# epfl-lts2/pygsp

Measured on AMD Instinct MI355X. Metric: filtered-vertices/sec (N·Nsig·K/s) + achieved HBM GB/s vs roofline, 1M-vertex K=30, higher is better.
Workload: dtype f64

## Files before the change

### pygsp_amd/csrc/gspx_ctx.hip.h

```cpp
#pragma once

struct Options {
  int64_t kernel = 0;
  int64_t vec = 0;
  int64_t rows_per_wave = 0;
  int64_t narrow_g_log2 = -1;
  int64_t waves_per_block = 4;
  int64_t calib_mix = 0;
  int64_t graph_launch = 2;
  int64_t tile_gather = 1;
  int64_t tile_workgroups = 0;
  int64_t knn_f32 = 1;
  int64_t tile_pad = 1;
  int64_t tile_min_row = 16;
  int64_t staged_copy = 1;
  int64_t staged_copy_min_mb = 32;
  int64_t copy_threads = 0;
  int64_t tile_regroup = 1;
  int64_t tile_lg = 0;
  int64_t edge_vertex_walk = 1;
  int64_t fuse_input = 1;
  int64_t tile_nt = -1;
  int64_t synthesis = 0;
  int64_t alternate_sweep = 1;
  int64_t xcd_remap = 1;
  int64_t combine = 0;
  int64_t ws_limit_mb = 65536;
  int64_t max_batch = 0;
  int64_t gather_rccl = 1;
  int64_t lds_pad_kb = 0;
  int64_t host_pipeline = 1;
  int64_t host_batch = 0;
  int64_t host_edge = 0;
  int64_t host_threads = 0;
  int64_t streamed_alloc = 1;
};

struct gspx_ctx {
  int device = 0;
  int cu_count = 256;
  hipStream_t stream = nullptr;
  Options opt;
  DevMem ws_t;
  DevMem ws_r;
  DevMem ws_w;
  DevMem io_x, io_y;
  DevMem ws_spec;
  DevMem ws_sq, ws_sqp;
  HostPipe* pipe = nullptr;
  CopyStage* copy = nullptr;
  bool counted = false;
  std::mutex comms_mu;
  std::vector<struct gspx_comm*> comms;
  hipEvent_t ev[4] = {nullptr, nullptr, nullptr, nullptr};
// ... 27 lines not shown
}

struct gspx_buf {
  gspx_ctx* ctx = nullptr;
  DevMem mem;
  int64_t bytes = 0;
};

static std::atomic<uint64_t> g_generation{1};

struct gspx_graph {
  gspx_ctx* ctx = nullptr;
  const uint64_t generation = g_generation.fetch_add(1);
  int64_t N = 0;
  int dtype = GSPX_F64;
  bool from_w = false;
  int64_t nnz_l = 0;
  DevMem lptr, lcol, lval, dw;
  int64_t nnz_int = 0;
  DevMem rptr, rcol, rval, fval, coff;
  unsigned coff_ldb = 0;
  DevMem perm, iperm;
  bool has_perm = false;
  double fval_lmax = -1.0;
  double build_ms = 0.0;
  bool has_bounds = false;
  double bounds[4] = {0, 0, 0, 0};
  DevMem gt_hdr, gt_s1rows, gt_lidx;
  DevMem gt_s1nat;
  int gt_ns1 = 0;
  int gt_rows = 0, gt_nb = 0, gt_slow = 0;
  size_t gt_lds = 0;
  int gt_entmax = 0;
  int lap_type = GSPX_LAP_COMBINATORIAL;
  bool edges_built = false;
  int64_t n_edges = 0;
  DevMem e_off, e_toff, e_src, e_dst, e_tedge, e_cs, e_ct, e_w;
};

static size_t elt_size(int dtype) { return dtype == GSPX_F32 ? 4 : 8; }

static hipEvent_t pool_event(gspx_ctx* ctx, size_t& i_ref) {
  size_t i = i_ref - 1;
  if (i >= 1024) {
    i = 1020 + (i & 3);
    i_ref = i + 1;
  }
  while (ctx->ev_pool.size() <= i) {
    hipEvent_t e = nullptr;
    if (hipEventCreate(&e) != hipSuccess) return nullptr;
    ctx->ev_pool.push_back(e);
  }
  return ctx->ev_pool[i];
}

extern "C" int gspx_device_count(int* n) {
  if (!n) return set_err(GSPX_ERR_INVALID, "gspx_device_count: null output");
  int c = 0;
  hipError_t e = hipGetDeviceCount(&c);
  if (e != hipSuccess) {
    *n = 0;
    (void)hipGetLastError();
    return set_err(GSPX_ERR_NODEVICE, "hipGetDeviceCount failed: %s", hipGetErrorString(e));
  }
  *n = c;
  return GSPX_OK;
// ... 100 lines not shown
}

struct OptionDef {
  const char* key;
  int64_t Options::*slot;
  bool (*ok)(int64_t);
  const char* refusal;
};
static const OptionDef OPTION_TABLE[] = {
    {"kernel", &Options::kernel, [](int64_t v) { return v == 0 || v == 1 || v == 2 || v == 5; },
     "kernel must be 0 (auto), 1 (panel), 2 (narrow) or 5 (LDS-staged)"},
    {"vec", &Options::vec, [](int64_t v) { return v == 0 || v == 1 || v == 2 || v == 4; }, "vec must be 0, 1, 2 or 4"},
    {"rows_per_wave", &Options::rows_per_wave, [](int64_t v) { return v >= 0 && v <= 1024; },
     "rows_per_wave must be in [0, 1024] (0 = auto)"},
    {"narrow_g_log2", &Options::narrow_g_log2, [](int64_t v) { return v >= -1 && v <= 6; },
     "narrow_g_log2 must be in [-1, 6] (-1 = auto)"},
    {"waves_per_block", &Options::waves_per_block, [](int64_t v) { return v == 4 || v == 8 || v == 16; },
     "waves_per_block must be 4, 8 or 16"},
    {"alternate_sweep", &Options::alternate_sweep, nullptr, nullptr},
    {"synthesis", &Options::synthesis, nullptr, nullptr},
    {"tile_gather", &Options::tile_gather, nullptr, nullptr},
    {"graph_launch", &Options::graph_launch, nullptr, nullptr},
    {"tile_workgroups", &Options::tile_workgroups, nullptr, nullptr},
    {"tile_lg", &Options::tile_lg, nullptr, nullptr},
    {"tile_regroup", &Options::tile_regroup, nullptr, nullptr},
    {"staged_copy", &Options::staged_copy, nullptr, nullptr},
    {"staged_copy_min_mb", &Options::staged_copy_min_mb, nullptr, nullptr},
    {"copy_threads", &Options::copy_threads, nullptr, nullptr},
    {"tile_min_row", &Options::tile_min_row, nullptr, nullptr},
    {"tile_pad", &Options::tile_pad, nullptr, nullptr},
    {"knn_f32", &Options::knn_f32, nullptr, nullptr},
    {"tile_nt", &Options::tile_nt, nullptr, nullptr},
    {"fuse_input", &Options::fuse_input, nullptr, nullptr},
    {"edge_vertex_walk", &Options::edge_vertex_walk, nullptr, nullptr},
    {"xcd_remap", &Options::xcd_remap, nullptr, nullptr},
    {"combine", &Options::combine, nullptr, nullptr},
    {"ws_limit_mb", &Options::ws_limit_mb, nullptr, nullptr},
    {"max_batch", &Options::max_batch, nullptr, nullptr},
    {"gather_rccl", &Options::gather_rccl, nullptr, nullptr},
    {"lds_pad_kb", &Options::lds_pad_kb, nullptr, nullptr},
    {"host_pipeline", &Options::host_pipeline, nullptr, nullptr},
    {"host_batch", &Options::host_batch, nullptr, nullptr},
    {"host_edge", &Options::host_edge, nullptr, nullptr},
    {"host_threads", &Options::host_threads, nullptr, nullptr},
    {"streamed_alloc", &Options::streamed_alloc, nullptr, nullptr},
};

static const OptionDef* find_option(const char* key) {
  if (key)
    for (const OptionDef& d : OPTION_TABLE)
      if (!strcmp(key, d.key)) return &d;
  set_err(GSPX_ERR_INVALID, "unknown option '%s'", key ? key : "(null)");
  return nullptr;
}

extern "C" int gspx_ctx_set_option(gspx_ctx* ctx, const char* key, int64_t value) {
  replay_reset(ctx);
  if (!ctx) return set_err(GSPX_ERR_INVALID, "null ctx");
  const OptionDef* d = find_option(key);
  if (!d) return GSPX_ERR_INVALID;
  if (d->ok && !d->ok(value)) return set_err(GSPX_ERR_INVALID, "%s", d->refusal);
  ctx->opt.*d->slot = value;
  if (d->slot == &Options::streamed_alloc) {
    const bool on = value != 0;
    (void)hipSetDevice(ctx->device);
    for (DevMem* m : {&ctx->ws_t, &ctx->ws_r}) {
// ... 186 lines not shown
```

### pygsp_amd/csrc/gspx_graph.hip.h

```cpp
#pragma once

namespace gspx {

#define GSPX_SCAN_TILE 1024
__global__ __launch_bounds__(256) void k_scan_tiles(const int* in, int n, int* out, int* __restrict__ tile_sums) {
  __shared__ int wsum[4];
  const int t = threadIdx.x, lane = t & 63, wv = t >> 6;
  const int base = blockIdx.x * GSPX_SCAN_TILE + t * 4;
  int v[4];
#pragma unroll
  for (int k = 0; k < 4; ++k) v[k] = (base + k < n) ? in[base + k] : 0;
  const int mine = v[0] + v[1] + v[2] + v[3];
  int incl = mine;
#pragma unroll
  for (int off = 1; off < 64; off <<= 1) {
    const int o = __shfl_up(incl, off);
    if (lane >= off) incl += o;
  }
  if (lane == 63) wsum[wv] = incl;
  __syncthreads();
  int wbase = 0;
  for (int k = 0; k < wv; ++k) wbase += wsum[k];
  int run = wbase + incl - mine;
#pragma unroll
// ... 615 lines not shown
  for (int i = 0; i < 4; ++i) out[i] = g->bounds[i];
  return GSPX_OK;
}

extern "C" int gspx_graph_download_internal(gspx_graph* g, int32_t* rowptr, int32_t* col) {
  if (!g || !rowptr) return set_err(GSPX_ERR_INVALID, "null argument");
  if (g->nnz_int > 0 && !col) return set_err(GSPX_ERR_INVALID, "null argument");
  HIPCHK(hipSetDevice(g->ctx->device));
  HIPCHK(hipMemcpy(rowptr, g->rptr.p, (size_t)(g->N + 1) * sizeof(int), hipMemcpyDeviceToHost));
  if (g->nnz_int > 0)
    HIPCHK(hipMemcpy(col, g->rcol.p, (size_t)g->nnz_int * sizeof(int), hipMemcpyDeviceToHost));
  return GSPX_OK;
}

extern "C" int gspx_graph_set_gather_tiles(gspx_graph* g, int block_rows, int nb, const int32_t* s1ptr,
                                           const int32_t* s1rows, const uint16_t* lidx, int64_t* stats) {
  if (g) replay_reset(g->ctx);
  if (!g) return set_err(GSPX_ERR_INVALID, "null graph");
  if (block_rows == 0) {
    g->gt_rows = 0;
    return GSPX_OK;
  }
  if (block_rows != GSPX_TILE_BR)
    return set_err(GSPX_ERR_INVALID, "gather tiles must use %d-row blocks", GSPX_TILE_BR);
  if (!s1ptr || !s1rows || !lidx || nb < 1 || nb != (int)((g->N + block_rows - 1) / block_rows))
    return set_err(GSPX_ERR_INVALID, "gspx_graph_set_gather_tiles: bad argument");
  HIPCHK(hipSetDevice(g->ctx->device));
  std::vector<int> rp((size_t)g->N + 1);
  HIPCHK(hipMemcpy(rp.data(), g->rptr.p, ((size_t)g->N + 1) * sizeof(int), hipMemcpyDeviceToHost));
  for (auto& r : rp) r &= ~3;
  const size_t lds = (size_t)52 * 1024;
  const size_t esz = elt_size(g->dtype);
  std::vector<int> hdr((size_t)nb * 4);
  int slow = 0, entmax = 0;
  for (int b = 0; b < nb; ++b) {
    const int lo = s1ptr[b], n1 = s1ptr[b + 1] - lo;
    const int r0 = b * block_rows, r1 = (int)std::min<int64_t>((int64_t)r0 + block_rows, g->N);
    const int ent = rp[r1] - rp[r0];
    if (n1 < 0 || lo < 0) return set_err(GSPX_ERR_INVALID, "gspx_graph_set_gather_tiles: bad s1ptr");
    for (int o = lo; o < lo + n1; ++o)
      if (s1rows[o] < 0 || s1rows[o] >= g->N)
        return set_err(GSPX_ERR_INVALID, "gspx_graph_set_gather_tiles: bad S1 row");
    const size_t need = (size_t)n1 * 256 + (((size_t)ent * esz + 15) & ~(size_t)15) +
                        (((size_t)ent * 2 + 15) & ~(size_t)15) + 32;
    const bool fast = n1 <= GSPX_TILE_MAXN1 && n1 < 65535 && need <= lds;
    slow += !fast;
    if (fast) entmax = std::max(entmax, ent);
    hdr[(size_t)b * 4 + 0] = lo;
    hdr[(size_t)b * 4 + 1] = fast ? n1 : -1;
    hdr[(size_t)b * 4 + 2] = rp[r0];
    hdr[(size_t)b * 4 + 3] = ent;
  }
  const int n_s1 = s1ptr[nb];
  CHK(g->gt_hdr.alloc(hdr.size() * 4 + 64));
  CHK(g->gt_s1rows.alloc((size_t)std::max(n_s1, 1) * 4 + 64));
  CHK(g->gt_lidx.alloc((size_t)g->nnz_int + 128));
  HIPCHK(hipMemcpy(g->gt_hdr.p, hdr.data(), hdr.size() * 4, hipMemcpyHostToDevice));
  HIPCHK(hipMemcpy(g->gt_s1rows.p, s1rows, (size_t)n_s1 * 4, hipMemcpyHostToDevice));
  {
    std::vector<unsigned char> l8((size_t)g->nnz_int);
    for (int b = 0; b < nb; ++b) {
      const bool fast = hdr[(size_t)b * 4 + 1] >= 0;
      const int e0 = hdr[(size_t)b * 4 + 2], e1 = e0 + hdr[(size_t)b * 4 + 3];
      for (int e = e0; e < e1; ++e) {
        if (fast && lidx[e] >= 256) return set_err(GSPX_ERR_INVALID, "gspx_graph_set_gather_tiles: tile position out of range");
        l8[(size_t)e] = fast ? (unsigned char)lidx[e] : 0;
      }
    }
    HIPCHK(hipMemcpy(g->gt_lidx.p, l8.data(), l8.size(), hipMemcpyHostToDevice));
  }
  g->gt_rows = block_rows;
  g->gt_nb = nb;
  g->gt_ns1 = n_s1;
  g->gt_s1nat.release();
  g->gt_slow = slow;
  g->gt_lds = lds;
  g->gt_entmax = entmax;
  if (stats) {
    stats[0] = nb;
    stats[1] = slow;
    stats[2] = (int64_t)lds;
  }
  return GSPX_OK;
}

static int build_tiles_dev(gspx_graph* g, size_t lds, DevMem& hdr, DevMem& s1rows, DevMem& lidx, int* out_nb, int* out_ns1,
                           int* out_slow, int* out_entmax) {
  gspx_ctx* ctx = g->ctx;
  hipStream_t st = ctx->stream;
  const int N = (int)g->N;
  constexpr int BR = GSPX_TILE_BR;
  const int nb = (N + BR - 1) / BR;
  DevMem tmp, n1, keep, s1lo, nslow;
  CHK(tmp.alloc((size_t)nb * GSPX_TILE_TMPCAP * sizeof(int)));
  CHK(n1.alloc(((size_t)nb + 1) * sizeof(int)));
  CHK(keep.alloc(((size_t)nb + 1) * sizeof(int)));
  CHK(s1lo.alloc(((size_t)nb + 1) * sizeof(int)));
  CHK(nslow.alloc(sizeof(int)));
  HIPCHK(hipMemsetAsync(nslow.p, 0, sizeof(int), st));
  hipLaunchKernelGGL(k_tiles_unique, dim3(nb), dim3(256), 0, st, g->rptr.as<int>(), g->rcol.as<int>(), N, nb,
                     tmp.as<int>(), n1.as<int>());
  hipLaunchKernelGGL(k_tiles_keep, dim3((nb + 1 + 255) / 256), dim3(256), 0, st, n1.as<int>(), nb,
                     keep.as<int>());
  CHK(scan_exclusive(ctx, keep.as<int>(), s1lo.as<int>(), nb + 1));
  int n_s1 = 0;
  HIPCHK(hipMemcpyAsync(&n_s1, s1lo.as<int>() + nb, sizeof(int), hipMemcpyDeviceToHost, st));
  HIPCHK(hipStreamSynchronize(st));
  CHK(hdr.alloc((size_t)nb * 4 * sizeof(int) + 64));
  CHK(s1rows.alloc((size_t)std::max(n_s1, 1) * 4 + 64));
  CHK(lidx.alloc((size_t)g->nnz_int + 128));
  hipLaunchKernelGGL(k_tiles_fill, dim3(nb), dim3(256), 0, st, g->rptr.as<int>(), g->rcol.as<int>(), N, nb,
                     tmp.as<int>(), n1.as<int>(), s1lo.as<int>(), (int)elt_size(g->dtype), (int)lds,
                     s1rows.as<int>(), lidx.as<unsigned char>(), hdr.as<int>(), nslow.as<int>());
  int slow = 0, entmax = 0;
  HIPCHK(hipMemcpyAsync(&slow, nslow.p, sizeof(int), hipMemcpyDeviceToHost, st));
  HIPCHK(hipMemsetAsync(nslow.p, 0, sizeof(int), st));
  hipLaunchKernelGGL(k_tiles_entmax, dim3((nb + 255) / 256), dim3(256), 0, st, hdr.as<int>(), nb, nslow.as<int>());
  HIPCHK(hipMemcpyAsync(&entmax, nslow.p, sizeof(int), hipMemcpyDeviceToHost, st));
  HIPCHK(hipGetLastError());
  HIPCHK(hipStreamSynchronize(st));
  *out_nb = nb;
  *out_ns1 = n_s1;
  *out_slow = slow;
  *out_entmax = entmax;
  return GSPX_OK;
}

extern "C" int gspx_graph_build_gather_tiles(gspx_graph* g, int64_t* stats) {
  if (!g) return set_err(GSPX_ERR_INVALID, "null graph");
  replay_reset(g->ctx);
  HIPCHK(hipSetDevice(g->ctx->device));
  if (g->N < 1) return set_err(GSPX_ERR_INVALID, "empty graph");
  const size_t lds = (size_t)52 * 1024;
  int nb = 0, n_s1 = 0, slow = 0, entmax = 0;
  CHK(build_tiles_dev(g, lds, g->gt_hdr, g->gt_s1rows, g->gt_lidx, &nb, &n_s1, &slow, &entmax));
  g->gt_rows = GSPX_TILE_BR;
  g->gt_nb = nb;
  g->gt_ns1 = n_s1;
  g->gt_s1nat.release();
  g->gt_slow = slow;
  g->gt_lds = lds;
  g->gt_entmax = entmax;
  if (stats) {
    stats[0] = nb;
    stats[1] = slow;
    stats[2] = (int64_t)lds;
    stats[3] = n_s1;
  }
  return GSPX_OK;
}

template <typename T> static int ensure_factor(gspx_graph* g, double lmax) {
  if (g->fval_lmax == lmax) return GSPX_OK;
  gspx_ctx* ctx = g->ctx;
  const int N = (int)g->N;
  const T a1 = (T)(lmax / 2.0), a2 = (T)(lmax / 2.0);
  const T two_over_a1 = T(2) / a1;
  const int nb = std::max(1, (N + 255) / 256);
  if (N > 0)
    hipLaunchKernelGGL((k_factor<T>), dim3(nb), dim3(256), 0, ctx->stream, g->rptr.as<int>(),
                       g->rcol.as<int>(), g->rval.as<T>(), N, two_over_a1, a2, g->fval.as<T>());
  HIPCHK(hipGetLastError());
  g->fval_lmax = lmax;
  return GSPX_OK;
}

__global__ void k_s1nat(const int* __restrict__ s1, const int* __restrict__ perm, int n, int* __restrict__ nat) {
  const int i = blockIdx.x * 256 + threadIdx.x;
  if (i < n) nat[i] = perm[s1[i]];
}
static int ensure_s1nat(gspx_graph* g, hipStream_t st) {
  if (g->gt_s1nat.p || !g->has_perm) return GSPX_OK;
  CHK(g->gt_s1nat.alloc((size_t)std::max(g->gt_ns1, 1) * 4 + 64));
  if (g->gt_ns1 > 0)
    hipLaunchKernelGGL(k_s1nat, dim3((g->gt_ns1 + 255) / 256), dim3(256), 0, st, g->gt_s1rows.as<int>(),
// ... 4 lines not shown
```

### pygsp_amd/csrc/gspx_poly.hip.h

```cpp
#pragma once

struct PlanStep {
  double scale = 1.0, gamma = -1.0;
  int flush = 0;
  int final = 0;
  std::vector<double> w;
};

static void make_plan_fused(int nf, int M, const std::vector<double>& cp, bool acc_existing,
                            bool final_to_y, std::vector<PlanStep>& plan) {
  const int K = M - 1;
  plan.assign((size_t)K, PlanStep());
  int covered = -1;
  bool first = !acc_existing;
  for (int k = 1; k <= K; ++k) {
    PlanStep& st = plan[(size_t)k - 1];
    st.scale = (k == 1) ? 0.5 : 1.0;
    st.gamma = (k == 1) ? 0.0 : -1.0;
    st.w.assign((size_t)nf * 3, 0.0);
    const bool must = (k == K) || (k >= 2 && (k - 2) > covered);
    if (!must) continue;
    st.flush = first ? 1 : 2;
    first = false;
    st.final = (k == K && final_to_y) ? 1 : 0;
// ... 306 lines not shown
       k_step_tile<T, 1, 4, true, false, 256>, k_step_tile<T, 1, 8, true>},
      {k_step_tile<T, 1, 1, false, true, 64>, k_step_tile<T, 1, 2, false, true, 128>,
       k_step_tile<T, 1, 4, false, true, 256>, k_step_tile<T, 1, 8, false, true>}};
  kern_t kern = narrow ? slim[flavour][lg == 1 ? 0 : lg == 2 ? 1 : lg == 4 ? 2 : 3] : wide[flavour][ncol <= 2 ? ncol : 0];
  unsigned threads = narrow ? 64u * (unsigned)lg : 512u;
  bool mix = false;
  if (opt.calib_mix && !narrow && flavour == 0) {
    static const kern_t mixk[2][3] = {
        {k_step_tile<T, 0, 16, false, false, 512, 16, 1>, k_step_tile<T, 1, 16, false, false, 512, 16, 1>,
         k_step_tile<T, 2, 16, false, false, 512, 16, 1>},
        {k_step_tile<T, 0, 16, false, false, 512, 16, 2>, k_step_tile<T, 1, 16, false, false, 512, 16, 2>,
         k_step_tile<T, 2, 16, false, false, 512, 16, 2>}};
    kern = mixk[opt.calib_mix == 2 ? 1 : 0][ncol <= 2 ? ncol : 0];
    mix = true;
  }
  const int pieces = (int)(rowb / 16);
  if (opt.tile_regroup && ncol == 1 && flavour != 1 && pieces < lg && !mix) {
#define GSPX_CL(LG_, CL_, NT_) \
  (flavour == 2 ? (kern_t)k_step_tile<T, 1, LG_, false, true, NT_, CL_> : (kern_t)k_step_tile<T, 1, LG_, false, false, NT_, CL_>)
    kern_t k2 = nullptr;
    unsigned nt2 = 0;
    if (lg == 4 && pieces == 3) k2 = GSPX_CL(4, 3, 192), nt2 = 192;
    else if (lg == 8 && pieces == 5) k2 = GSPX_CL(8, 5, 320), nt2 = 320;
    else if (lg == 16 && pieces == 10) k2 = GSPX_CL(16, 10, 320), nt2 = 320;
#undef GSPX_CL
    if (k2) kern = k2, threads = nt2;
  }
  size_t lds = g->gt_lds;
  if (lg < 8)
    lds = std::min(lds, (size_t)GSPX_TILE_MAXN1 * 16 * lg + (((size_t)g->gt_entmax * sizeof(T) + 15) & ~(size_t)15) +
                            (((size_t)g->gt_entmax + 15) & ~(size_t)15) + 64);
  if (lg < 8) lds = (lds + 2047) & ~(size_t)2047;
  int per_cu = 2;
  {
    struct Known { size_t attr = 0; std::map<size_t, int> fit; };
    static std::map<std::pair<const void*, int>, Known> known;
    static std::mutex lds_mu;
    std::lock_guard<std::mutex> lock(lds_mu);
    Known& k = known[std::make_pair((const void*)kern, g->ctx->device)];
    if (k.attr < lds) {
      HIPCHK(hipFuncSetAttribute((const void*)kern, hipFuncAttributeMaxDynamicSharedMemorySize, (int)lds));
      k.attr = lds;
    }
    if (lg < 8) {
      auto it = k.fit.find(lds);
      if (it == k.fit.end()) {
        int fit = 2;
        HIPCHK(hipOccupancyMaxActiveBlocksPerMultiprocessor(&fit, (const void*)kern, (int)threads, lds));
        it = k.fit.emplace(lds, std::max(2, std::min(fit, 16))).first;
      }
      per_cu = it->second;
    }
  }
  t.rowptr = g->rptr.as<int>();
  t.col = g->rcol.as<int>();
  t.val = vals ? vals : g->fval.as<T>();
  t.hdr = g->gt_hdr.as<int>();
  if (!t.s1rows) t.s1rows = g->gt_s1rows.as<int>();
  t.lidx = g->gt_lidx.as<unsigned char>();
  t.N = (int)g->N;
  t.ld = ld;
  t.panel_bytes = (unsigned)((size_t)g->N * ld * sizeof(T));
  t.val_bytes = (unsigned)((size_t)g->nnz_int * sizeof(T));
  t.lidx_bytes = (unsigned)((size_t)g->nnz_int);
  t.nb = g->gt_nb;
  t.ncol = ncol;
  t.per_xcd = (t.nb + 7) / 8;
  t.lds_bytes = (int)lds;
  unsigned nwg = (unsigned)std::max<int64_t>(8, ((int64_t)per_cu * g->ctx->cu_count) / 8 * 8);
  if (opt.tile_workgroups > 0)
    nwg = (unsigned)std::max<int64_t>(8, std::min<int64_t>(opt.tile_workgroups, 1 << 20) / 8 * 8);
  nwg = std::min(nwg, 8u * (unsigned)std::max(t.per_xcd, 1));
  t.nt = opt.tile_nt >= 0 ? (int)opt.tile_nt : ((size_t)g->N * ld * sizeof(T) >= ((size_t)192 << 20) ? 5 : 0);
  hipLaunchKernelGGL(kern, dim3(nwg), dim3(threads), lds, st, t);
  return GSPX_OK;
}

template <typename T>
static int prepare_coff(gspx_graph* g, const Shape& shape, unsigned ld, hipStream_t st) {
  if (shape.kernel == 5 && g->coff_ldb != ld * (unsigned)sizeof(T)) {
    CHK(g->coff.ensure(((size_t)g->nnz_int + 64) * sizeof(unsigned)));
    const int nb = std::max(1, (int)((g->N + 255) / 256));
    hipLaunchKernelGGL((k_coff<T>), dim3(nb), dim3(256), 0, st, g->rptr.as<int>(), g->rcol.as<int>(), (int)g->N,
                       ld * (unsigned)sizeof(T), g->coff.as<unsigned>());
    g->coff_ldb = ld * (unsigned)sizeof(T);
// ... 309 lines not shown
      a.gamma = T(0);
    } else {
      a.cur = B[(k + 1) & 1];
      a.out = B[k & 1];
      const bool has_b2 = (k + 2 <= K);
      a.old = has_b2 ? B[k & 1] : a.cur;
      a.gamma = has_b2 ? T(-1) : T(0);
      a.scale = (k == 0) ? T(0.5) : T(1);
    }
    a.reverse = (opt.alternate_sweep && (k & 1)) ? 1 : 0;
    launch_step<T>(a, shape, opt, st, g->coff.as<unsigned>());
  }
  HIPCHK(hipEventRecord(ev[2], st));
  if (padded) {
    const unsigned nbp = (unsigned)std::min<size_t>(((size_t)N * ld + 255) / 256, 65536);
    hipLaunchKernelGGL((k_permute_out_pad<T>), dim3(nbp), dim3(256), 0, st, B[0], ldw, y, ldy, ld, N, perm);
  }
  HIPCHK(hipEventRecord(ev[3], st));
  HIPCHK(hipGetLastError());
  return GSPX_OK;
}

template <typename T>
static int run_program_batch(gspx_graph* g, int S, const double* sc, const double* be, const double* ga, bool old_is_x,
                             const T* x, unsigned ldx, T* y, unsigned ldy, unsigned ld, size_t& ev_idx) {
  gspx_ctx* ctx = g->ctx;
  Options opt = ctx->opt;
  hipStream_t st = ctx->stream;
  const int N = (int)g->N;
  const size_t U = (size_t)N * ld;
  const Shape shape = choose_shape(opt, sizeof(T), ld, vec_cap(4, ldy, y));
  const int* perm = g->has_perm ? g->perm.as<int>() : nullptr;

  const T hw[3] = {T(1), T(0), T(0)};
  CHK(ctx->ws_w.ensure(sizeof(hw) + 64));
  HIPCHK(hipMemcpyAsync(ctx->ws_w.p, hw, sizeof(hw), hipMemcpyHostToDevice, st));
  HIPCHK(hipStreamSynchronize(st));
  CHK(ctx->ws_t.ensure((old_is_x ? 3 : 2) * U * sizeof(T) + 256));
  T* X = ctx->ws_t.as<T>();
  T* H[2] = {X + U, old_is_x ? X + 2 * U : X};

  hipEvent_t ev[4];
  CHK(batch_events(ctx, ev_idx, ev));
  launch_permute_in<T>(x, ldx, X, ld, N, perm, vec_cap(shape.vec, ldx, x), st);
  HIPCHK(hipEventRecord(ev[1], st));

  CHK(prepare_coff<T>(g, shape, ld, st));
  StepArgs<T> a = step_base<T>(g, ld, y, ldy);
  a.nf = 1;
  a.racc = H[0];
  a.wts = ctx->ws_w.as<T>();
  const bool tile_ok = tile_usable<T>(g, opt, ld, y, ldy);
  for (int s = 0; s < S; ++s) {
    const bool last = s == S - 1;
    const T* cur = (s == 0) ? X : H[(s - 1) & 1];
    T* out = H[s & 1];
    const T* old = old_is_x ? X : (const T*)out;
    const double gam = (!old_is_x && s == 0) ? 0.0 : ga[s];
    if (tile_ok) {
      TileArgs<T> t{};
      t.cur = cur;
      t.old = gam == 0.0 ? cur : old;
      t.out = out;
      t.racc = H[0];
      t.y = y;
      t.ldy = ldy;
      t.perm = perm;
      t.scale = (T)sc[s];
      t.beta = (T)be[s];
      t.gamma = (T)gam;
      t.flush = 0;
      t.final = last ? 1 : 0;
      t.reverse = (opt.alternate_sweep && (s & 1)) ? 1 : 0;
      CHK(launch_step_tile<T>(g, opt, t, ld, st));
      continue;
    }
    a.cur = cur;
    a.old = gam == 0.0 ? cur : old;
    a.out = out;
    a.scale = (T)sc[s];
    a.beta = (T)be[s];
    a.gamma = (T)gam;
    a.flush = last ? 1 : 0;
    a.final = last ? 1 : 0;
    a.reverse = (opt.alternate_sweep && (s & 1)) ? 1 : 0;
    launch_step<T>(a, shape, opt, st, g->coff.as<unsigned>());
  }
  HIPCHK(hipEventRecord(ev[2], st));
  HIPCHK(hipEventRecord(ev[3], st));
  HIPCHK(hipGetLastError());
  return GSPX_OK;
}

template <typename T>
static int filter_dev_t(gspx_graph* g, double lmax, int Nf, int M, const double* coeffs,
                        int64_t Nsig, const T* x, T* y, int mode) {
  gspx_ctx* ctx = g->ctx;
  const Options& opt = ctx->opt;
  const int64_t N = g->N;
  for (int i = 0; i < 5; ++i) ctx->timing[i] = 0;
  if (N == 0 || Nsig == 0) return GSPX_OK;
  CHK(ensure_factor<T>(g, lmax));
  std::vector<double> cp;
  halve_c0(Nf, M, coeffs, cp);

  const int K = M - 1;
// ... 347 lines not shown
```

### pygsp_amd/csrc/gspx_tile_kernels.hip.h

```cpp
#pragma once

#include "gspx_kernels.hip.h"

namespace gspx {

template <typename T> struct TileArgs {
  const int* rowptr;
  const int* col;
  const T* val;
  const int* hdr;
  const int* s1rows;
  const u8* lidx;
  const T* cur;
  const T* old;
  const int* old_rows;
  T* out;
  T* racc;
  T* y;
  const int* perm;
  int N;
  u32 ld, ldy;
  u32 panel_bytes, val_bytes, lidx_bytes;
  int nb, ncol, per_xcd;
  int lds_bytes;
  T scale, gamma;
  T beta;
  T wn, wc, wo;
  const T* inp;
  const T* wts;
  int nin;
  int flush;
  int final;
  int reverse;
  int nt;
};

constexpr int GSPX_TILE_BR = 64;
constexpr int GSPX_TILE_MAXN1 = 160;

template <typename T, int NCOL, int LG, bool OLDNAT> struct TileSchedule {
  static constexpr bool PF = !OLDNAT;
  static constexpr bool TILE_LAST = PF && LG == 16;
  static constexpr bool PF_ENTRIES = PF;
  static constexpr bool META_AFTER = !OLDNAT && LG == 16 && NCOL == 0;
};

template <typename T, int NCOL, int LG = 16, bool OLDNAT = false, bool INS = false, int NT = 512, int CL = LG,
          int MIX = 0>
__global__ __launch_bounds__(NT, 4) void k_step_tile(const TileArgs<T> a) {
  static_assert(NT == 512 || (NT == 64 * LG && NCOL == 1) || (CL < LG && NCOL == 1 && NT % 64 == 0 && NT % CL == 0),
                "narrow builds: one row per group, one chunk per row");
  constexpr int BR = GSPX_TILE_BR;
  static_assert(CL <= LG && (BR % (NT / CL)) == 0, "compute groups must tile the block's rows");
  constexpr int MAXN1 = GSPX_TILE_MAXN1;
  constexpr bool PF = TileSchedule<T, NCOL, LG, OLDNAT>::PF;
  constexpr bool META_AFTER = TileSchedule<T, NCOL, LG, OLDNAT>::META_AFTER;
  constexpr bool TILE_LAST = TileSchedule<T, NCOL, LG, OLDNAT>::TILE_LAST;
  constexpr bool PF_ENTRIES = TileSchedule<T, NCOL, LG, OLDNAT>::PF_ENTRIES;
  constexpr int VEC = 16 / (int)sizeof(T);
  typedef typename VT<T, VEC>::t V;
  typedef __attribute__((address_space(3))) void* lds_ptr;
  extern __shared__ __attribute__((aligned(16))) unsigned char gspx_smem[];

  const int tid = threadIdx.x;
  constexpr int NGD = NT / LG;
  constexpr int NG = NT / CL;
  constexpr int NE = (512 + NT - 1) / NT;
  constexpr int RPG = BR / NG;
  constexpr int ST = (MAXN1 + NGD - 1) / NGD;
  constexpr int RB = LG * 16;
  const int lane_d = tid & (LG - 1);
  const int grp_d = tid / LG;
  const int lane16 = CL == LG ? lane_d : tid % CL;
  const int grp = CL == LG ? grp_d : tid / CL;
  const int wave = tid >> 6;
  const int nwx = (int)(gridDim.x >> 3);
  const int xlo = (int)(blockIdx.x & 7) * a.per_xcd;
  int k1 = xlo + a.per_xcd;
  if (k1 > a.nb) k1 = a.nb;
  const int k0 = xlo + (int)(blockIdx.x >> 3);
  if (k0 >= k1) return;

  constexpr u32 POISON = 0x80000000u;
  const rsrc_t rcur = __builtin_amdgcn_make_buffer_rsrc((void*)a.cur, 0, a.panel_bytes, 0x00020000);
// ... 19 lines not shown
    const int n1 = h.y;
#pragma unroll
    for (int t = 0; t < ST; ++t) {
      const int u = grp_d + NGD * t;
      m.rows[t] = a.s1rows[h.x + (u < n1 ? u : 0)];
    }
    int r = phys(k) * BR + grp * RPG;
#pragma unroll
    for (int t = 0; t < RPG + 1; ++t) m.rp[t] = a.rowptr[(r + t) <= a.N ? (r + t) : a.N];
    if constexpr (OLDNAT) {
#pragma unroll
      for (int t = 0; t < RPG; ++t) m.orow[t] = a.old_rows[(r + t) < a.N ? (r + t) : a.N - 1];
    }
    return m;
  };
  V* const tile = (V*)gspx_smem;
  auto stage = [&](const Meta& m, int n1, u32 cb) {
#pragma unroll
    for (int t = 0; t < ST; ++t) {
      if (grp_d + NGD * t < n1)
        __builtin_amdgcn_raw_ptr_buffer_load_lds(rcur, (lds_ptr)(gspx_smem + (wave * (64 / LG) + NGD * t) * RB), 16,
                                                 (u32)m.rows[t] * ldb + cb, 0, 0, 0);
    }
  };
  auto chunk_off_d = [&](int c) {
    const u32 col0 = (c * LG + lane_d) * VEC;
    return col0 < a.ld ? col0 * (u32)sizeof(T) : POISON;
  };
  auto chunk_off = [&](int c) {
    const u32 col0 = (c * LG + lane16) * VEC;
    return col0 < a.ld ? col0 * (u32)sizeof(T) : POISON;
  };

  V ov[RPG], ra[RPG];
  u32x4 ev[NE], ei = 0;
#pragma unroll
  for (int q = 0; q < NE; ++q) ev[q] = 0;
  auto prefetch_rows = [&](const Meta& m, int blk, int c) {
    const int r0 = phys(blk) * BR + grp * RPG;
    const u32 cb = chunk_off(c);
#pragma unroll
    for (int t = 0; t < RPG; ++t) {
      const u32 off = (r0 + t < a.N && cb != POISON) ? (u32)(r0 + t) * ldb + cb : POISON;
      u32 oo = a.gamma != T(0) ? off : POISON;
      if constexpr (OLDNAT) oo = (off != POISON && a.gamma != T(0)) ? (u32)m.orow[t] * ldb + cb : POISON;
      if (a.nt & 4) ov[t] = __builtin_bit_cast(V, __builtin_amdgcn_raw_buffer_load_b128(rold, oo, 0, 2));
      else ov[t] = VT<T, VEC>::bload(rold, oo);
      const u32 ro = a.flush == 2 ? off : POISON;
      if (a.nt & 2) ra[t] = __builtin_bit_cast(V, __builtin_amdgcn_raw_buffer_load_b128(rra, ro, 0, 2));
      else ra[t] = VT<T, VEC>::bload(rra, ro);
    }
  };
  auto prefetch_entries = [&](const int4& h) {
    const int nv16 = (h.w * (int)sizeof(T) + 15) >> 4, ni16 = (h.w + 15) >> 4;
    const u32 io = tid < ni16 ? (u32)h.z + tid * 16u : POISON;
#pragma unroll
    for (int q = 0; q < NE; ++q) {
      const int i = tid + q * NT;
      const u32 vo = i < nv16 ? (u32)h.z * (u32)sizeof(T) + i * 16u : POISON;
      if (a.nt & 1) ev[q] = __builtin_amdgcn_raw_buffer_load_b128(rv, vo, 0, 2);
      else ev[q] = __builtin_amdgcn_raw_buffer_load_b128(rv, vo, 0, 0);
    }
    if (a.nt & 1) ei = __builtin_amdgcn_raw_buffer_load_b128(ri, io, 0, 2);
    else ei = __builtin_amdgcn_raw_buffer_load_b128(ri, io, 0, 0);
  };

  int4 H = uniform(load_hdr(k0));
  Meta M = load_meta(k0, H);
  int k = k0, kn = k0 + nwx, knn = k0 + 2 * nwx;
  int4 Hn = uniform(load_hdr(kn < k1 ? kn : k0));
  if constexpr (!TILE_LAST) {
    if (H.y >= 0) stage(M, H.y, chunk_off_d(0));
  }
  if constexpr (PF) prefetch_rows(M, k0, 0);
  if constexpr (PF_ENTRIES) {
// ... 28 lines not shown
#pragma unroll
        for (int t = 0; t < RPG; ++t) {
          const u32 off = (row0 + t < a.N) ? (u32)(row0 + t) * ldb + cb : POISON;
          ins[t] += w * VT<T, VEC>::bload(rin, off == POISON ? POISON : off + (u32)f * a.panel_bytes);
        }
      }
    }
    if constexpr (!PF_ENTRIES) {
      if (first && fast) prefetch_entries(H);
    }
    int4 Hv = Hn;
    if constexpr (!META_AFTER) {
      if (last) {
        M = load_meta(kn < k1 ? kn : k, Hn);
        Hv = load_hdr(knn < k1 ? knn : k);
      }
    }
    __builtin_amdgcn_sched_barrier(0);
    if (first && fast) {
      const int nv16 = (ent * (int)sizeof(T) + 15) >> 4, ni16 = (ent + 15) >> 4;
#pragma unroll
      for (int q = 0; q < NE; ++q)
        if (tid + q * NT < nv16) *(u32x4*)((unsigned char*)mval + (tid + q * NT) * 16) = ev[q];
      if (tid < ni16) *(u32x4*)((unsigned char*)midx + tid * 16) = ei;
      for (int i = tid + NE * NT; i < nv16; i += NT)
        *(u32x4*)((unsigned char*)mval + i * 16) =
            __builtin_amdgcn_raw_buffer_load_b128(rv, (u32)rp0 * (u32)sizeof(T) + i * 16u, 0, 0);
      for (int i = tid + NT; i < ni16; i += NT)
        *(u32x4*)((unsigned char*)midx + i * 16) =
            __builtin_amdgcn_raw_buffer_load_b128(ri, (u32)rp0 + i * 16u, 0, 0);
    }
    if constexpr (TILE_LAST && !META_AFTER) {
      constexpr int NMETA = ST + RPG + 1 + 1;
      static_assert(NMETA < 16, "vmcnt immediate");
      if (last && !INS) __builtin_amdgcn_s_waitcnt(0x0070 | NMETA);
      else __builtin_amdgcn_s_waitcnt(0x0070);
    } else {
      __builtin_amdgcn_s_waitcnt(0x0070);
    }
    if constexpr (MIX != 2) __syncthreads();
    if constexpr (META_AFTER) {
      if (last) {
        M = load_meta(kn < k1 ? kn : k, Hn);
        Hv = load_hdr(knn < k1 ? knn : k);
      }
    }
    __builtin_amdgcn_sched_barrier(0);
    V nv[RPG], res[RPG];
#pragma unroll
    for (int t = 0; t < RPG; ++t) {
      const int s = rs[t], e = rs[t + 1];
      V acc = 0, self = 0;
      if (MIX && fast) {
        self = tile[(int)midx[s - rp0] * LG + lane16];
        acc = mval[s - rp0] * self;
      } else if (fast) {
        acc = lds_row_dot<T, V, LG, u8>(mval + (s - rp0), midx + (s - rp0), row0 + t < a.N ? e - s : 0, tile, lane16,
                                        self);
      } else if (row0 + t < a.N) {
        for (int j = s; j < e; ++j) {
          const int cc = a.col[j];
          const V xv = VT<T, VEC>::bload(rcur, cc < a.N ? (u32)cc * ldb + cb : POISON);
          if (j == s) self = xv;
          acc += a.val[j] * xv;
        }
      }
      nv[t] = a.scale * acc + a.gamma * ov[t] + a.beta * self;
      if constexpr (INS) nv[t] += ins[t];
      res[t] = a.wn * nv[t] + a.wc * self + a.wo * ov[t];
      if (a.flush == 2) res[t] += ra[t];
    }
    __builtin_amdgcn_s_waitcnt(0xC07F);
    if constexpr (MIX != 2) __builtin_amdgcn_s_barrier();
    bool more = true;
    if (last) {
      const int4 Hnn = uniform(Hv);
      H = Hn;
      Hn = Hnn;
      more = kn < k1;
    }
    __builtin_amdgcn_sched_barrier(0);
    if constexpr (!PF) {
      if (more && H.y >= 0) stage(M, H.y, chunk_off_d(last ? 0 : c + 1));
    }
#pragma unroll
    for (int t = 0; t < RPG; ++t) {
      const int row = row0 + t;
      if (row < a.N && on) {
        if (a.final && !a.flush) {
          const size_t orow = a.perm ? (size_t)a.perm[row] : (size_t)row;
          *(V*)(a.y + orow * a.ldy + col0) = nv[t];
          continue;
        }
        if (a.nt & 8) __builtin_nontemporal_store(nv[t], (V*)(a.out + (size_t)row * a.ld + col0));
        else *(V*)(a.out + (size_t)row * a.ld + col0) = nv[t];
        if (a.flush) {
          if (a.final) {
            const size_t orow = a.perm ? (size_t)a.perm[row] : (size_t)row;
            *(V*)(a.y + orow * a.ldy + col0) = res[t];
          } else {
            if (a.nt & 2) __builtin_nontemporal_store(res[t], (V*)(a.racc + (size_t)row * a.ld + col0));
            else *(V*)(a.racc + (size_t)row * a.ld + col0) = res[t];
          }
        }
      }
    }
    __builtin_amdgcn_sched_barrier(0);
    if constexpr (PF) {
      if (more) {
        const int nc = last ? 0 : c + 1;
        if constexpr (!TILE_LAST) {
          if (H.y >= 0) stage(M, H.y, chunk_off_d(nc));
        }
        prefetch_rows(M, last ? kn : k, nc);
        if constexpr (PF_ENTRIES) {
          if (last && H.y >= 0) prefetch_entries(H);
        }
        if constexpr (TILE_LAST) {
          __builtin_amdgcn_sched_barrier(0);
          if (H.y >= 0) stage(M, H.y, chunk_off_d(nc));
          __builtin_amdgcn_sched_barrier(0);
        }
      }
    }
    if (last) {
      k = kn;
      kn = knn;
      knn += nwx;
    }
    return more;
  };
  for (;;) {
    if constexpr (NCOL == 1) {
      if (!pass(0, true, true)) break;
    } else if constexpr (NCOL == 2) {
// ... 84 lines not shown
  const int r0 = b * BR, r1 = min(r0 + BR, N);
  const int e0 = rowptr[r0] & ~3, e1 = rowptr[r1] & ~3;
  const int ent = e1 - e0;
  const int n = n1[b];
  const long need = (long)n * ROWB + (((long)ent * esz + 15) & ~15L) + (((long)ent * 2 + 15) & ~15L) + 32;
  const bool fast = n <= MAXN1 && need <= lds_bytes;
  const int lo = s1lo[b];
  if (threadIdx.x == 0) {
    hdr[(size_t)b * 4 + 0] = lo;
    hdr[(size_t)b * 4 + 1] = fast ? n : -1;
    hdr[(size_t)b * 4 + 2] = e0;
    hdr[(size_t)b * 4 + 3] = ent;
    if (!fast) atomicAdd(nslow, 1);
  }
  const int* list = tmp + (size_t)b * GSPX_TILE_TMPCAP;
  const int keep = n <= GSPX_TILE_TMPCAP ? n : 0;
  for (int i = threadIdx.x; i < keep; i += 256) s1rows[lo + i] = list[i];
  for (int i = threadIdx.x; i < ent; i += 256) {
    const int c = col[e0 + i];
    int pos = 0;
    if (c < N && fast) {
      int a = 0, z = n;
      while (a < z) {
        const int mid = (a + z) >> 1;
        if (list[mid] < c) a = mid + 1; else z = mid;
      }
      pos = a;
    }
    lidx[e0 + i] = (u8)pos;
  }
}
__global__ void k_tiles_entmax(const int* __restrict__ hdr, int nb, int* __restrict__ out) {
  const int b = blockIdx.x * 256 + threadIdx.x;
  if (b < nb && hdr[(size_t)b * 4 + 1] >= 0) atomicMax(out, hdr[(size_t)b * 4 + 3]);
}

__global__ void k_tiles_keep(const int* __restrict__ n1, int nb, int* __restrict__ keep) {
  const int b = blockIdx.x * blockDim.x + threadIdx.x;
  if (b <= nb) keep[b] = (b < nb && n1[b] <= GSPX_TILE_TMPCAP) ? n1[b] : 0;
}

}
```

Before: 186.1 billion.

## Add two-panel 256-thread tile kernel variant and fuse input permute into first step

Adds a specialised 256-thread tile-step kernel (TWO template flag) for plain steps with no old-term, flush or mixing. It drops the per-row old and accumulator registers and sizes LDS from the actual maximum S1 row count, which is now tracked during tile build. If the occupancy query reports at least three blocks per CU, this kernel replaces the default 512-thread one. Separately, when tiles are usable the input permute kernel is skipped and the first step reads x directly through natural-order S1 rows, and the weights upload and sync are skipped. The cost is more template instantiations, a vmcnt encoding change, and a dependency on the new n1max bookkeeping being correct.

Result: no change. 186.6 billion (median of 4 runs) (+0.3%).

```diff
diff --git a/pygsp_amd/csrc/gspx_ctx.hip.h b/pygsp_amd/csrc/gspx_ctx.hip.h
--- a/pygsp_amd/csrc/gspx_ctx.hip.h
+++ b/pygsp_amd/csrc/gspx_ctx.hip.h
@@ -20,6 +20,7 @@
   int64_t tile_lg = 0;
   int64_t edge_vertex_walk = 1;
   int64_t fuse_input = 1;
+  int64_t tile_two_panel = 1;
   int64_t tile_nt = -1;
   int64_t synthesis = 0;
   int64_t alternate_sweep = 1;
@@ -113,6 +114,7 @@
   int gt_rows = 0, gt_nb = 0, gt_slow = 0;
   size_t gt_lds = 0;
   int gt_entmax = 0;
+  int gt_n1max = 0;
   int lap_type = GSPX_LAP_COMBINATORIAL;
   bool edges_built = false;
   int64_t n_edges = 0;
@@ -279,6 +281,7 @@
     {"knn_f32", &Options::knn_f32, nullptr, nullptr},
     {"tile_nt", &Options::tile_nt, nullptr, nullptr},
     {"fuse_input", &Options::fuse_input, nullptr, nullptr},
+    {"tile_two_panel", &Options::tile_two_panel, [](int64_t v) { return v == 0 || v == 1; }, "tile_two_panel must be 0 or 1"},
     {"edge_vertex_walk", &Options::edge_vertex_walk, nullptr, nullptr},
     {"xcd_remap", &Options::xcd_remap, nullptr, nullptr},
     {"combine", &Options::combine, nullptr, nullptr},
diff --git a/pygsp_amd/csrc/gspx_graph.hip.h b/pygsp_amd/csrc/gspx_graph.hip.h
--- a/pygsp_amd/csrc/gspx_graph.hip.h
+++ b/pygsp_amd/csrc/gspx_graph.hip.h
@@ -671,7 +671,7 @@
   const size_t lds = (size_t)52 * 1024;
   const size_t esz = elt_size(g->dtype);
   std::vector<int> hdr((size_t)nb * 4);
-  int slow = 0, entmax = 0;
+  int slow = 0, entmax = 0, n1max = 0;
   for (int b = 0; b < nb; ++b) {
     const int lo = s1ptr[b], n1 = s1ptr[b + 1] - lo;
     const int r0 = b * block_rows, r1 = (int)std::min<int64_t>((int64_t)r0 + block_rows, g->N);
@@ -684,7 +684,7 @@
                         (((size_t)ent * 2 + 15) & ~(size_t)15) + 32;
     const bool fast = n1 <= GSPX_TILE_MAXN1 && n1 < 65535 && need <= lds;
     slow += !fast;
-    if (fast) entmax = std::max(entmax, ent);
+    if (fast) entmax = std::max(entmax, ent), n1max = std::max(n1max, n1);
     hdr[(size_t)b * 4 + 0] = lo;
     hdr[(size_t)b * 4 + 1] = fast ? n1 : -1;
     hdr[(size_t)b * 4 + 2] = rp[r0];
@@ -715,6 +715,7 @@
   g->gt_slow = slow;
   g->gt_lds = lds;
   g->gt_entmax = entmax;
+  g->gt_n1max = n1max;
   if (stats) {
     stats[0] = nb;
     stats[1] = slow;
@@ -724,7 +725,7 @@
 }
 
 static int build_tiles_dev(gspx_graph* g, size_t lds, DevMem& hdr, DevMem& s1rows, DevMem& lidx, int* out_nb, int* out_ns1,
-                           int* out_slow, int* out_entmax) {
+                           int* out_slow, int* out_entmax, int* out_n1max) {
   gspx_ctx* ctx = g->ctx;
   hipStream_t st = ctx->stream;
   const int N = (int)g->N;
@@ -735,8 +736,8 @@
   CHK(n1.alloc(((size_t)nb + 1) * sizeof(int)));
   CHK(keep.alloc(((size_t)nb + 1) * sizeof(int)));
   CHK(s1lo.alloc(((size_t)nb + 1) * sizeof(int)));
-  CHK(nslow.alloc(sizeof(int)));
-  HIPCHK(hipMemsetAsync(nslow.p, 0, sizeof(int), st));
+  CHK(nslow.alloc(2 * sizeof(int)));
+  HIPCHK(hipMemsetAsync(nslow.p, 0, 2 * sizeof(int), st));
   hipLaunchKernelGGL(k_tiles_unique, dim3(nb), dim3(256), 0, st, g->rptr.as<int>(), g->rcol.as<int>(), N, nb,
                      tmp.as<int>(), n1.as<int>());
   hipLaunchKernelGGL(k_tiles_keep, dim3((nb + 1 + 255) / 256), dim3(256), 0, st, n1.as<int>(), nb,
@@ -751,17 +752,18 @@
   hipLaunchKernelGGL(k_tiles_fill, dim3(nb), dim3(256), 0, st, g->rptr.as<int>(), g->rcol.as<int>(), N, nb,
                      tmp.as<int>(), n1.as<int>(), s1lo.as<int>(), (int)elt_size(g->dtype), (int)lds,
                      s1rows.as<int>(), lidx.as<unsigned char>(), hdr.as<int>(), nslow.as<int>());
-  int slow = 0, entmax = 0;
+  int slow = 0, maxes[2] = {0, 0};
   HIPCHK(hipMemcpyAsync(&slow, nslow.p, sizeof(int), hipMemcpyDeviceToHost, st));
-  HIPCHK(hipMemsetAsync(nslow.p, 0, sizeof(int), st));
+  HIPCHK(hipMemsetAsync(nslow.p, 0, 2 * sizeof(int), st));
   hipLaunchKernelGGL(k_tiles_entmax, dim3((nb + 255) / 256), dim3(256), 0, st, hdr.as<int>(), nb, nslow.as<int>());
-  HIPCHK(hipMemcpyAsync(&entmax, nslow.p, sizeof(int), hipMemcpyDeviceToHost, st));
+  HIPCHK(hipMemcpyAsync(maxes, nslow.p, 2 * sizeof(int), hipMemcpyDeviceToHost, st));
   HIPCHK(hipGetLastError());
   HIPCHK(hipStreamSynchronize(st));
   *out_nb = nb;
   *out_ns1 = n_s1;
   *out_slow = slow;
-  *out_entmax = entmax;
+  *out_entmax = maxes[0];
+  *out_n1max = maxes[1];
   return GSPX_OK;
 }
 
@@ -771,8 +773,8 @@
   HIPCHK(hipSetDevice(g->ctx->device));
   if (g->N < 1) return set_err(GSPX_ERR_INVALID, "empty graph");
   const size_t lds = (size_t)52 * 1024;
-  int nb = 0, n_s1 = 0, slow = 0, entmax = 0;
-  CHK(build_tiles_dev(g, lds, g->gt_hdr, g->gt_s1rows, g->gt_lidx, &nb, &n_s1, &slow, &entmax));
+  int nb = 0, n_s1 = 0, slow = 0, entmax = 0, n1max = 0;
+  CHK(build_tiles_dev(g, lds, g->gt_hdr, g->gt_s1rows, g->gt_lidx, &nb, &n_s1, &slow, &entmax, &n1max));
   g->gt_rows = GSPX_TILE_BR;
   g->gt_nb = nb;
   g->gt_ns1 = n_s1;
@@ -780,6 +782,7 @@
   g->gt_slow = slow;
   g->gt_lds = lds;
   g->gt_entmax = entmax;
+  g->gt_n1max = n1max;
   if (stats) {
     stats[0] = nb;
     stats[1] = slow;
diff --git a/pygsp_amd/csrc/gspx_poly.hip.h b/pygsp_amd/csrc/gspx_poly.hip.h
--- a/pygsp_amd/csrc/gspx_poly.hip.h
+++ b/pygsp_amd/csrc/gspx_poly.hip.h
@@ -362,25 +362,45 @@
                             (((size_t)g->gt_entmax + 15) & ~(size_t)15) + 64);
   if (lg < 8) lds = (lds + 2047) & ~(size_t)2047;
   int per_cu = 2;
-  {
+  auto prepare = [&](kern_t kn, unsigned nthr, size_t bytes, bool ask_fit, int* fit_out) -> int {
     struct Known { size_t attr = 0; std::map<size_t, int> fit; };
     static std::map<std::pair<const void*, int>, Known> known;
     static std::mutex lds_mu;
     std::lock_guard<std::mutex> lock(lds_mu);
-    Known& k = known[std::make_pair((const void*)kern, g->ctx->device)];
-    if (k.attr < lds) {
-      HIPCHK(hipFuncSetAttribute((const void*)kern, hipFuncAttributeMaxDynamicSharedMemorySize, (int)lds));
-      k.attr = lds;
-    }
-    if (lg < 8) {
-      auto it = k.fit.find(lds);
+    Known& k = known[std::make_pair((const void*)kn, g->ctx->device)];
+    if (k.attr < bytes) {
+      HIPCHK(hipFuncSetAttribute((const void*)kn, hipFuncAttributeMaxDynamicSharedMemorySize, (int)bytes));
+      k.attr = bytes;
+    }
+    if (ask_fit) {
+      auto it = k.fit.find(bytes);
       if (it == k.fit.end()) {
         int fit = 2;
-        HIPCHK(hipOccupancyMaxActiveBlocksPerMultiprocessor(&fit, (const void*)kern, (int)threads, lds));
-        it = k.fit.emplace(lds, std::max(2, std::min(fit, 16))).first;
+        HIPCHK(hipOccupancyMaxActiveBlocksPerMultiprocessor(&fit, (const void*)kn, (int)nthr, bytes));
+        it = k.fit.emplace(bytes, std::min(fit, 16)).first;
       }
-      per_cu = it->second;
-    }
+      *fit_out = it->second;
+    }
+    return GSPX_OK;
+  };
+  bool two = false;
+  if (opt.tile_two_panel && t.gamma == T(0) && !t.flush && t.nin == 0 && !t.old_rows && !mix && !narrow &&
+      kern == wide[0][ncol <= 2 ? ncol : 0]) {
+    static const kern_t twok[3] = {k_step_tile<T, 0, 16, false, false, 256, 16, 0, true>,
+                                   k_step_tile<T, 1, 16, false, false, 256, 16, 0, true>,
+                                   k_step_tile<T, 2, 16, false, false, 256, 16, 0, true>};
+    const kern_t k2 = twok[ncol <= 2 ? ncol : 0];
+    size_t lds2 = (size_t)g->gt_n1max * 256 + (((size_t)g->gt_entmax * sizeof(T) + 15) & ~(size_t)15) +
+                  (((size_t)g->gt_entmax + 15) & ~(size_t)15) + 64;
+    lds2 = std::min(lds, (lds2 + 2047) & ~(size_t)2047);
+    int fit = 0;
+    CHK(prepare(k2, 256u, lds2, true, &fit));
+    if (fit >= 3) kern = k2, threads = 256u, lds = lds2, per_cu = fit, two = true;
+  }
+  if (!two) {
+    int fit = 2;
+    CHK(prepare(kern, threads, lds, lg < 8, &fit));
+    if (lg < 8) per_cu = std::max(2, fit);
   }
   t.rowptr = g->rptr.as<int>();
   t.col = g->rcol.as<int>();
@@ -756,17 +776,29 @@
   const Shape shape = choose_shape(opt, sizeof(T), ld, vec_cap(4, ldy, y));
   const int* perm = g->has_perm ? g->perm.as<int>() : nullptr;
 
+  const bool tile_ok = tile_usable<T>(g, opt, ld, y, ldy);
   const T hw[3] = {T(1), T(0), T(0)};
-  CHK(ctx->ws_w.ensure(sizeof(hw) + 64));
-  HIPCHK(hipMemcpyAsync(ctx->ws_w.p, hw, sizeof(hw), hipMemcpyHostToDevice, st));
-  HIPCHK(hipStreamSynchronize(st));
+  if (!tile_ok) {
+    CHK(ctx->ws_w.ensure(sizeof(hw) + 64));
+    HIPCHK(hipMemcpyAsync(ctx->ws_w.p, hw, sizeof(hw), hipMemcpyHostToDevice, st));
+    HIPCHK(hipStreamSynchronize(st));
+  }
   CHK(ctx->ws_t.ensure((old_is_x ? 3 : 2) * U * sizeof(T) + 256));
   T* X = ctx->ws_t.as<T>();
   T* H[2] = {X + U, old_is_x ? X + 2 * U : X};
 
   hipEvent_t ev[4];
   CHK(batch_events(ctx, ev_idx, ev));
-  launch_permute_in<T>(x, ldx, X, ld, N, perm, vec_cap(shape.vec, ldx, x), st);
+  const unsigned char* xb = (const unsigned char*)x;
+  const unsigned char* yb = (const unsigned char*)y;
+  const size_t xbytes = (size_t)N * ldx * sizeof(T), ybytes = (size_t)N * ldy * sizeof(T);
+  const bool fuse_in = tile_ok && !old_is_x && opt.fuse_input && g->gt_slow == 0 && ldx == ld &&
+                       ((uintptr_t)x % 16) == 0 && (xb + xbytes <= yb || yb + ybytes <= xb) &&
+                       (!g->has_perm || g->gt_ns1 > 0);
+  if (fuse_in)
+    CHK(ensure_s1nat(g, st));
+  else
+    launch_permute_in<T>(x, ldx, X, ld, N, perm, vec_cap(shape.vec, ldx, x), st);
   HIPCHK(hipEventRecord(ev[1], st));
 
   CHK(prepare_coff<T>(g, shape, ld, st));
@@ -774,7 +806,6 @@
   a.nf = 1;
   a.racc = H[0];
   a.wts = ctx->ws_w.as<T>();
-  const bool tile_ok = tile_usable<T>(g, opt, ld, y, ldy);
   for (int s = 0; s < S; ++s) {
     const bool last = s == S - 1;
     const T* cur = (s == 0) ? X : H[(s - 1) & 1];
@@ -796,6 +827,14 @@
       t.flush = 0;
       t.final = last ? 1 : 0;
       t.reverse = (opt.alternate_sweep && (s & 1)) ? 1 : 0;
+      if (fuse_in && s == 0) {
+        t.cur = x;
+        t.old = x;
+        t.s1rows = g->has_perm ? g->gt_s1nat.as<int>() : nullptr;
+      } else if (fuse_in && s == 1 && gam != 0.0) {
+        t.old = x;
+        t.old_rows = perm;
+      }
       CHK(launch_step_tile<T>(g, opt, t, ld, st));
       continue;
     }
diff --git a/pygsp_amd/csrc/gspx_tile_kernels.hip.h b/pygsp_amd/csrc/gspx_tile_kernels.hip.h
--- a/pygsp_amd/csrc/gspx_tile_kernels.hip.h
+++ b/pygsp_amd/csrc/gspx_tile_kernels.hip.h
@@ -46,10 +46,13 @@
 };
 
 template <typename T, int NCOL, int LG = 16, bool OLDNAT = false, bool INS = false, int NT = 512, int CL = LG,
-          int MIX = 0>
-__global__ __launch_bounds__(NT, 4) void k_step_tile(const TileArgs<T> a) {
-  static_assert(NT == 512 || (NT == 64 * LG && NCOL == 1) || (CL < LG && NCOL == 1 && NT % 64 == 0 && NT % CL == 0),
+          int MIX = 0, bool TWO = false>
+__global__ __launch_bounds__(NT, TWO ? 3 : 4) void k_step_tile(const TileArgs<T> a) {
+  static_assert(NT == 512 || (NT == 64 * LG && NCOL == 1) || (CL < LG && NCOL == 1 && NT % 64 == 0 && NT % CL == 0) ||
+                    (TWO && NT == 256 && LG == 16),
                 "narrow builds: one row per group, one chunk per row");
+  static_assert(!TWO || (NT == 256 && LG == 16 && CL == 16 && !OLDNAT && !INS && MIX == 0),
+                "two-panel build: 256 threads, 16-lane groups, plain flavour");
   constexpr int BR = GSPX_TILE_BR;
   static_assert(CL <= LG && (BR % (NT / CL)) == 0, "compute groups must tile the block's rows");
   constexpr int MAXN1 = GSPX_TILE_MAXN1;
@@ -135,7 +138,7 @@
     return col0 < a.ld ? col0 * (u32)sizeof(T) : POISON;
   };
 
-  V ov[RPG], ra[RPG];
+  V ov[TWO ? 1 : RPG], ra[TWO ? 1 : RPG];
   u32x4 ev[NE], ei = 0;
 #pragma unroll
   for (int q = 0; q < NE; ++q) ev[q] = 0;
@@ -143,7 +146,7 @@
     const int r0 = phys(blk) * BR + grp * RPG;
     const u32 cb = chunk_off(c);
 #pragma unroll
-    for (int t = 0; t < RPG; ++t) {
+    for (int t = 0; t < (TWO ? 0 : RPG); ++t) {
       const u32 off = (r0 + t < a.N && cb != POISON) ? (u32)(r0 + t) * ldb + cb : POISON;
       u32 oo = a.gamma != T(0) ? off : POISON;
       if constexpr (OLDNAT) oo = (off != POISON && a.gamma != T(0)) ? (u32)m.orow[t] * ldb + cb : POISON;
@@ -238,8 +241,8 @@
     }
     if constexpr (TILE_LAST && !META_AFTER) {
       constexpr int NMETA = ST + RPG + 1 + 1;
-      static_assert(NMETA < 16, "vmcnt immediate");
-      if (last && !INS) __builtin_amdgcn_s_waitcnt(0x0070 | NMETA);
+      static_assert(NMETA < 64, "vmcnt immediate");
+      if (last && !INS) __builtin_amdgcn_s_waitcnt(0x0070 | (NMETA & 15) | ((NMETA >> 4) << 14));
       else __builtin_amdgcn_s_waitcnt(0x0070);
     } else {
       __builtin_amdgcn_s_waitcnt(0x0070);
@@ -252,7 +255,7 @@
       }
     }
     __builtin_amdgcn_sched_barrier(0);
-    V nv[RPG], res[RPG];
+    V nv[RPG], res[TWO ? 1 : RPG];
 #pragma unroll
     for (int t = 0; t < RPG; ++t) {
       const int s = rs[t], e = rs[t + 1];
@@ -271,10 +274,14 @@
           acc += a.val[j] * xv;
         }
       }
-      nv[t] = a.scale * acc + a.gamma * ov[t] + a.beta * self;
-      if constexpr (INS) nv[t] += ins[t];
-      res[t] = a.wn * nv[t] + a.wc * self + a.wo * ov[t];
-      if (a.flush == 2) res[t] += ra[t];
+      if constexpr (TWO) {
+        nv[t] = a.scale * acc + a.gamma * V(0) + a.beta * self;
+      } else {
+        nv[t] = a.scale * acc + a.gamma * ov[t] + a.beta * self;
+        if constexpr (INS) nv[t] += ins[t];
+        res[t] = a.wn * nv[t] + a.wc * self + a.wo * ov[t];
+        if (a.flush == 2) res[t] += ra[t];
+      }
     }
     __builtin_amdgcn_s_waitcnt(0xC07F);
     if constexpr (MIX != 2) __builtin_amdgcn_s_barrier();
@@ -293,20 +300,22 @@
     for (int t = 0; t < RPG; ++t) {
       const int row = row0 + t;
       if (row < a.N && on) {
-        if (a.final && !a.flush) {
+        if (a.final && (TWO || !a.flush)) {
           const size_t orow = a.perm ? (size_t)a.perm[row] : (size_t)row;
           *(V*)(a.y + orow * a.ldy + col0) = nv[t];
           continue;
         }
         if (a.nt & 8) __builtin_nontemporal_store(nv[t], (V*)(a.out + (size_t)row * a.ld + col0));
         else *(V*)(a.out + (size_t)row * a.ld + col0) = nv[t];
-        if (a.flush) {
-          if (a.final) {
-            const size_t orow = a.perm ? (size_t)a.perm[row] : (size_t)row;
-            *(V*)(a.y + orow * a.ldy + col0) = res[t];
-          } else {
-            if (a.nt & 2) __builtin_nontemporal_store(res[t], (V*)(a.racc + (size_t)row * a.ld + col0));
-            else *(V*)(a.racc + (size_t)row * a.ld + col0) = res[t];
+        if constexpr (!TWO) {
+          if (a.flush) {
+            if (a.final) {
+              const size_t orow = a.perm ? (size_t)a.perm[row] : (size_t)row;
+              *(V*)(a.y + orow * a.ldy + col0) = res[t];
+            } else {
+              if (a.nt & 2) __builtin_nontemporal_store(res[t], (V*)(a.racc + (size_t)row * a.ld + col0));
+              else *(V*)(a.racc + (size_t)row * a.ld + col0) = res[t];
+            }
           }
         }
       }
@@ -457,7 +466,10 @@
 }
 __global__ void k_tiles_entmax(const int* __restrict__ hdr, int nb, int* __restrict__ out) {
   const int b = blockIdx.x * 256 + threadIdx.x;
-  if (b < nb && hdr[(size_t)b * 4 + 1] >= 0) atomicMax(out, hdr[(size_t)b * 4 + 3]);
+  if (b < nb && hdr[(size_t)b * 4 + 1] >= 0) {
+    atomicMax(out, hdr[(size_t)b * 4 + 3]);
+    atomicMax(out + 1, hdr[(size_t)b * 4 + 1]);
+  }
 }
 
 __global__ void k_tiles_keep(const int* __restrict__ n1, int nb, int* __restrict__ keep) {
```
